# pelinski/TransformerGrooveInfilling

Hardware: AMD Instinct MI355X
Metric: HVO sequences/sec (32-step, d_model=128) per train step (higher is better)
Workload: dtype f32; 1 GPU; BASELINE configs[1]: InfillingClosedHH_training.yaml + overrides d_model=128/4 heads/3 layers, dim_feedforward=512, bs=64 per GPU, dropout=0.24, SGD lr=0.07, hit_loss_penalty=0.38, S=16, encoder-only; global_batch=64, parallelism=dp1, hipgraph=False

## Files before the change

transformergrooveinfilling_amd/csrc/gt_seq.h:

```cpp
#pragma once
#include "gt_seq_api.h"
#include <type_traits>

#ifdef GT_SEQ_STAMPS
#define GT_STAMP(i) do { if (blockIdx.x == 0 && threadIdx.x == 0) reinterpret_cast<long long*>(a.ws + a.stamps)[(i)] = (long long)__builtin_amdgcn_s_memtime(); } while (0)
__shared__ long long* gt_sub_ptr;
#define GT_SUBSTAMP(i) do { if (threadIdx.x == 0 && gt_sub_ptr) gt_sub_ptr[(i)] = (long long)__builtin_amdgcn_s_memtime(); } while (0)
#define GT_SUBWAIT() asm volatile("s_waitcnt vmcnt(0) lgkmcnt(0)" ::: "memory")
#define GT_SUBSET(on) do { if (threadIdx.x == 0) gt_sub_ptr = ((on) && blockIdx.x == 0) ? reinterpret_cast<long long*>(a.ws + a.stamps) + 200 : nullptr; } while (0)
#define GT_WGSTAMP(k) do { if (threadIdx.x == 0 && a.phase == 1 && blockIdx.x < 512) { long long* q_ = reinterpret_cast<long long*>(a.ws + a.stamps) + 1024 + 4 * blockIdx.x + 2 * (k); \
    q_[0] = (long long)__builtin_amdgcn_s_memtime(); q_[1] = (long long)__builtin_amdgcn_s_memrealtime(); } } while (0)
#else
#define GT_WGSTAMP(k) do { } while (0)
#define GT_STAMP(i) do { } while (0)
#define GT_SUBSTAMP(i) do { } while (0)
#define GT_SUBWAIT() do { } while (0)
#define GT_SUBSET(on) do { } while (0)
#endif

#define GT_SEQ_WAVES 8
#define GT_SEQ_NT (GT_SEQ_WAVES * 64)
#define GT_SEQ_NT_WG GT_SEQ_NT
#include "gt_seq_wg.h"

// ... 78 lines not shown
      w[j] = __hip_atomic_load(slot + j * GT_SEQ_NT + tid, __ATOMIC_RELAXED, __HIP_MEMORY_SCOPE_AGENT);
      ok = ok && (uint32_t)(w[j] >> 32) == GT_XTAG;
    }
    if (__all(ok)) break;
    if (spins == 0 && __hip_atomic_load(err, __ATOMIC_RELAXED, __HIP_MEMORY_SCOPE_AGENT) != 0u) spins = spin_max;
    if (++spins > spin_max) { if ((tid & 63) == 0) __hip_atomic_store(err, 1u, __ATOMIC_RELAXED, __HIP_MEMORY_SCOPE_AGENT); break; }
    __builtin_amdgcn_s_sleep(1);
  }
#pragma unroll
  for (int j = 0; j < 4; ++j) __hip_atomic_store(slot + j * GT_SEQ_NT + tid, 0ull, __ATOMIC_RELAXED, __HIP_MEMORY_SCOPE_AGENT);
#endif
  return f32x4{gt_u2f((uint32_t)w[0]), gt_u2f((uint32_t)w[1]), gt_u2f((uint32_t)w[2]), gt_u2f((uint32_t)w[3])};
}


template <bool BKM, bool VEC>
__device__ __forceinline__ void seq_ldb(float (&b)[4], const float* __restrict__ W, const int ldw, const int n, const int N, const int k,
                                        const int K, const float* zp) {
  if (!BKM && VEC) {
    const float4 v = *reinterpret_cast<const float4*>((n < N && k < K) ? W + (size_t)n * ldw + k : zp);
    b[0] = v.x; b[1] = v.y; b[2] = v.z; b[3] = v.w;
  } else if (!BKM) {
#pragma unroll
    for (int j = 0; j < 4; ++j) b[j] = *((n < N && k + j < K) ? W + (size_t)n * ldw + k + j : zp);
  } else {
#pragma unroll
    for (int j = 0; j < 4; ++j) b[j] = *((n < N && k + j < K) ? W + (size_t)(k + j) * ldw + n : zp);
  }
}
template <bool HALF>
__device__ __forceinline__ void seq_mma(f32x4& acc0, f32x4& acc1, const float (&b)[4], const float* sA, const int lda, const int l16, const int k) {
  const float4 a0 = *reinterpret_cast<const float4*>(sA + l16 * lda + k);
  acc0 = GT_MFMA16(b[0], a0.x, acc0); acc0 = GT_MFMA16(b[1], a0.y, acc0); acc0 = GT_MFMA16(b[2], a0.z, acc0); acc0 = GT_MFMA16(b[3], a0.w, acc0);
  if (!HALF) {
    const float4 a1 = *reinterpret_cast<const float4*>(sA + (16 + l16) * lda + k);
    acc1 = GT_MFMA16(b[0], a1.x, acc1); acc1 = GT_MFMA16(b[1], a1.y, acc1); acc1 = GT_MFMA16(b[2], a1.z, acc1); acc1 = GT_MFMA16(b[3], a1.w, acc1);
  }
}
template <bool BKM, bool VEC, int NK, bool HALF, typename Epi>
__device__ __forceinline__ void seq_mm_edge(const float* sA, const int lda, const int K, const float* __restrict__ W, const int ldw, const int N,
                                            const float* __restrict__ bias, const int wave, const int lane, const float* zp, Epi epi) {
  const int l16 = lane & 15, lg = lane >> 4;
  const int n0 = wave * 16;
  if (n0 >= N) return;
  float b[NK][4], bi[4];
#pragma unroll
  for (int u = 0; u < NK; ++u) { if (16 * u < K) seq_ldb<BKM, VEC>(b[u], W, ldw, n0 + l16, N, 16 * u + 4 * lg, K, zp); }
#pragma unroll
  for (int r = 0; r < 4; ++r) bi[r] = *((bias != nullptr && n0 + 4 * lg + r < N) ? bias + n0 + 4 * lg + r : zp);
  f32x4 acc0 = f32x4{0.f, 0.f, 0.f, 0.f}, acc1 = f32x4{0.f, 0.f, 0.f, 0.f};
#pragma unroll
  for (int u = 0; u < NK; ++u) { if (16 * u < K) seq_mma<HALF>(acc0, acc1, b[u], sA, lda, l16, 16 * u + 4 * lg); }
  epi(n0, acc0, acc1, bi);
}

template <int NK> struct SeqB { float4 v[NK]; };
template <int NK, bool FULL = false>
__device__ __forceinline__ void seq_b_load(SeqB<NK>& b, const float* __restrict__ Wp, const int nkt, const int t, const int u0, const int nk,
                                           const int lane) {
  const float* p = Wp + (unsigned)(((t * nkt + u0) * 64 + lane) * 4);
#pragma unroll
  for (int u = 0; u < NK; ++u) { if (FULL || u < nk) b.v[u] = *reinterpret_cast<const float4*>(p + 256 * u); }
}
#ifdef GT_SEQ_TU_FWD
__global__ __launch_bounds__(256) void seq_pack_kernel(SeqArgs a) {
  const int lane = threadIdx.x & 63, l16 = lane & 15, lg = lane >> 4;
  const int d = a.d, F = a.F, d16 = d >> 4, f16 = F >> 4;
  const int nf0 = 3 * d16 * d16, nf1 = d16 * d16, nf2 = f16 * d16, T = nf0 + nf1 + 2 * nf2;
  const int g = blockIdx.x * 4 + (threadIdx.x >> 6);
  if (g >= 2 * a.L * T) return;
  const int pack = g / (a.L * T), r = g % (a.L * T), l = r / T;
  int f = r % T, R, C;
  int64_t src, moff;
  if (f < nf0) { src = a.p0.in_w; R = 3 * d; C = d; moff = 0; }
  else if (f < nf0 + nf1) { f -= nf0; src = a.p0.out_w; R = d; C = d; moff = (int64_t)3 * d * d; }
  else if (f < nf0 + nf1 + nf2) { f -= nf0 + nf1; src = a.p0.w1; R = F; C = d; moff = (int64_t)4 * d * d; }
  else { f -= nf0 + nf1 + nf2; src = a.p0.w2; R = d; C = F; moff = (int64_t)4 * d * d + (int64_t)d * F; }
  const float* W = a.prm + src + (int64_t)l * a.pstride;
  float4 v;
  if (pack == 0) {
    const int nkt = C >> 4, t = f / nkt, u = f % nkt;
    v = *reinterpret_cast<const float4*>(W + (size_t)(16 * t + l16) * C + 16 * u + 4 * lg);
  } else {
    const int nkt = R >> 4, t = f / nkt, u = f % nkt;
    const float* p = W + (size_t)(16 * u + 4 * lg) * C + 16 * t + l16;
    v = make_float4(p[0], p[C], p[2 * (size_t)C], p[3 * (size_t)C]);
  }
  *reinterpret_cast<float4*>(a.ws + (pack ? a.pack_b : a.pack_f) + (int64_t)l * a.kstride + moff + (int64_t)f * 256 + lane * 4) = v;
}

struct SeqUpd { float* prm; float* g; float* m; float* v; int64_t n; const gt_step_state* st; int algo, step_advanced, nblk_a; const unsigned* err; };
__device__ __forceinline__ float seq_upd_elem(const SeqUpd& u, const int64_t i, const float w, const float g, const float k, const float b1,
                                              const float b2, const float step_size, const float inv_sqrt_bc2, const float gs, const float eps,
                                              const bool skip) {
  if (skip) return w;
  if (u.algo == 0) return w - k * g;
  const float gi = g * gs;
  const float mi = b1 * u.m[i] + (1.0f - b1) * gi;
  const float vi = b2 * u.v[i] + (1.0f - b2) * gi * gi;
  u.m[i] = mi; u.v[i] = vi;
  return w - step_size * mi / (sqrtf(vi) * inv_sqrt_bc2 + eps);
}
__global__ __launch_bounds__(256) void seq_update_pack_kernel(SeqArgs a, SeqUpd u) {
  __shared__ float tr[4][16][17];
  const int lane = threadIdx.x & 63, wave = threadIdx.x >> 6, l16 = lane & 15, lg = lane >> 4;
  const float k = u.st->lr * u.st->grad_scale;
// ... 867 lines not shown
  if (tid >= 2 * nkrow * H) return;
  const int pb = tid & 1, jb = krow0 + (tid >> 1) % nkrow, hb = (tid >> 1) / nkrow;
  const float msc = dk.thr ? dk.scale : 1.0f;
  const int i0 = 16 * pb;
  const float* qp = sQ + hb * HD + i0 * ldq;
  const float* dop = sDO + hb * HD + i0 * lddo;
  const float* rdp = srd + hb * 32 + i0;
  const uint32_t* mwp = reinterpret_cast<const uint32_t*>(srd) + H * 32 + hb * 32 + i0;
  const float* pim = sImg + (4 * pb) * 2048 + (4 * hb) * 32 + 4 * ((jb >> 2) ^ (hb & 7)) + (jb & 3);
  const int hx = hb >> 3;
  const SeqHv<HD> v = seq_hv_ld<HD>(sQ + jb * ldq + 2 * d + hb * HD);
  const uint32_t allk = dk.thr ? 0u : 1u;
#pragma unroll
  for (int i = 0; i < 16; ++i) {
    const float pi = pim[(i >> 2) * 2048 + ((i & 3) ^ hx) * 32];
    const float mk = (((mwp[i] >> jb) | allk) & 1u) ? msc : 0.f;
    const SeqHv<HD> dO = seq_hv_ld<HD>(dop + i * lddo), qi = seq_hv_ld<HD>(qp + i * ldq);
    const float pm = pi * mk, g = pi * (seq_hv_dot<HD>(dO, v) * mk - rdp[i]) * scale;
#pragma unroll
    for (int c = 0; c < HD; ++c) { G.dvv.v[c] += pm * dO.v[c]; G.dkk.v[c] += g * qi.v[c]; }
    if ((i & 3) == 3) { GT_SCHED_FENCE() }
  }
#pragma unroll
  for (int c = 0; c < HD; ++c) { G.dvv.v[c] += seq_lane_swap1(G.dvv.v[c]); G.dkk.v[c] += seq_lane_swap1(G.dkk.v[c]); }
}
template <int HD>
__device__ __forceinline__ void seq_attn_bwd_small_store(const SeqAttnSmallG<HD>& G, float* sQ, const int ldq, const int d, const int H,
                                                         const int krow0, const int nkrow, const int tid) {
  if (tid < 32 * H) {
    const int ha = tid % H, ia = tid / H;
#pragma unroll
    for (int c = 0; c < HD; ++c) sQ[ia * ldq + ha * HD + c] = G.dq.v[c];
  }
  if (tid < 2 * nkrow * H) {
    const int pb = tid & 1, jb = krow0 + (tid >> 1) % nkrow, hb = (tid >> 1) / nkrow;
    float* dst = sQ + jb * ldq + (pb ? 2 * d : d) + hb * HD;
#pragma unroll
    for (int c = 0; c < HD; ++c) dst[c] = pb ? G.dvv.v[c] : G.dkk.v[c];
  }
}

__device__ __forceinline__ int seq_vblock(const int bid, const int nper, const int B) {
  if ((B & 7) != 0 || bid >= nper * B) return bid;
  const int xcd = bid & 7, slot = bid >> 3;
  return ((slot / nper) * 8 + xcd) * nper + slot % nper;
}

template <int DP> struct SeqGeo {
  static constexpr int SX = DP + 8, SH = GT_SEQ_FMAX + 8, SQ = 3 * DP + 8, SRS = DP + 8, RP = DP == 32 ? 8 : DP == 64 ? 2 : 1, CW = DP / 16;
  static constexpr int TILE = 32 * SX, QKV = 32 * SQ, FFN = 32 * SH, RES = RP * 32 * SRS, NK = DP / 16;
  static constexpr int UNI = QKV > FFN ? QKV : FFN;
};
template <int DP> struct SeqFwdLds { static constexpr int N = 3 * SeqGeo<DP>::TILE + SeqGeo<DP>::RES + SeqGeo<DP>::UNI; };
template <int DP, int HDC, bool EXACT, bool SPLIT, bool QUAD = false>
__device__ __forceinline__ bool seq_fwd_body(const SeqArgs& a, float* const lds) {
  static_assert(!QUAD || (SPLIT && EXACT && DP == 128), "QUAD: the SPLIT kernels of d_model 128");
  using G = SeqGeo<DP>;
  constexpr int SX = G::SX, SH = G::SH, SQ = G::SQ, SRS = G::SRS, CW = G::CW, NK = G::NK;
  constexpr int HD = SeqHd<HDC>::HD;
  constexpr bool PAD = SeqHd<HDC>::PAD;
  constexpr bool HALF = SPLIT;
  constexpr int NH = HALF ? 1 : 2, NROW = HALF ? 16 : 32;
  float* const sX = lds; float* const sX1 = sX + G::TILE; float* const sC = sX1 + G::TILE; float* const sR = sC + G::TILE; float* const sU = sR + G::RES;
  float* const sQ = sU;
  float* const sH = sU;
  const int tid = threadIdx.x, lane = tid & 63, wave = tid >> 6, l16 = lane & 15, lg = lane >> 4;
  const int vb = (SPLIT && !QUAD) ? seq_vblock((int)blockIdx.x, 2, a.B) : (int)blockIdx.x;
  const int cpart = QUAD ? (vb & 1) : 0;
  const int half_id = QUAD ? (vb >> 1) : vb;
  const int b = SPLIT ? half_id >> 1 : (int)blockIdx.x, rb = SPLIT ? 16 * (half_id & 1) : 0;
  const bool sv0 = !QUAD || cpart == 0, sv1 = !QUAD || cpart == 1;
  const int d = EXACT ? DP : a.d, F = a.F;
  const size_t r0 = (size_t)b * 32;
  const float* const zp = gt_zero_ptr();
  const float* prm = a.prm;
  float* ws = a.ws;
  const SeqDropK dk = seq_dropk(a);
  const uint32_t idxd = (uint32_t)(r0 * d), idxf = (uint32_t)(r0 * F);
  const float ascale = 1.0f / sqrtf((float)a.hd);
  constexpr bool PF32 = SPLIT && !QUAD && EXACT && (DP == 32 || DP == 64);
  constexpr bool PFLN = PF32;
  SeqB<NK> ipre = SeqB<NK>();
  float4 ipre_b = make_float4(0.f, 0.f, 0.f, 0.f);
  bool have_ipre = false;
  auto load_rows = [&](float* dst, const int str, const float* src, const int ncol, const int rb_, const int nrows) {
    const int q4 = ncol >> 2;
    for (int e = tid; e < nrows * q4; e += GT_SEQ_NT) {
      const int r = rb_ + e / q4, c = (e % q4) * 4;
      *reinterpret_cast<float4*>(dst + r * str + c) = *reinterpret_cast<const float4*>(src + (unsigned)(r * ncol + c));
    }
  };

  auto input_layer = [&](auto all_tag) {
    constexpr bool HF = HALF && !decltype(all_tag)::value;
    constexpr int NHX = HF ? 1 : 2, NRX = HF ? 16 : 32;
    const int rbx = HF ? rb : 0;
    for (int e = tid; e < NRX * 32; e += GT_SEQ_NT) {
      const int r = rbx + (e >> 5), c = e & 31;
      sC[r * SX + c] = *(c < a.S ? a.xin + (r0 + r) * a.S + c : zp);
    }
    GT_BARRIER();
    GT_STAMP(1);
    const uint32_t key = seq_key(dk, GT_SITE_PE_ENC);
    float* ga0 = ws + a.a0 + r0 * d;
    float* gx0 = ws + a.x0 + r0 * d;
    seq_mm_edge<false, false, 2, HF>(sC + rbx * SX, SX, a.S, prm + a.in_w, a.S, d, prm + a.in_b, wave, lane, zp,
                                     [&](int n0, const f32x4& c0, const f32x4& c1, const float (&bi)[4]) {
#pragma unroll
      for (int h2 = 0; h2 < NHX; ++h2) {
// ... 163 lines not shown
    GT_BARRIER();
    GT_SUBSET(false);
    GT_STAMP(sb + 5);
    if constexpr (QUAD) {
      seq_tile_out_cols(wl + a.w0.hact + r0 * F, F, sH, SH, fc0, fcn, tid, rb, NROW);
      f32x4 acc0 = f32x4{0.f, 0.f, 0.f, 0.f}, acc1 = acc0;
      seq_mm_krange<true>(acc0, acc1, sH + rb * SH + l16 * SH + 4 * lg, SH, kf_w2, nkf, wave, kq0, kq0 + (nkf >> 1), lane, pre2, b2pre);
      GT_STAMP(300 + 4 * l);
      unsigned long long* const xq = reinterpret_cast<unsigned long long*>(ws + a.xchg) + 8;
      const bool last = l + 1 == a.L;
      const bool fz = a.fuse_b0 != 0;
      if (!last || cpart == 1 || fz) seq_xchg_put(xq + (size_t)vb * GT_XCHG_WG_GRANULES, acc0, tid);
      if (last && cpart == 1 && !fz) return true;
      *reinterpret_cast<float4*>(&sR[(16 * cpart + l16) * SRS + 16 * wave + 4 * lg]) = make_float4(acc0[0], acc0[1], acc0[2], acc0[3]);
      GT_STAMP(301 + 4 * l);
      const f32x4 oth = seq_xchg_get(xq + (size_t)(vb ^ 1) * GT_XCHG_WG_GRANULES, tid, reinterpret_cast<unsigned*>(ws + a.xchg), a.spin_max);
      GT_STAMP(302 + 4 * l);
      *reinterpret_cast<float4*>(&sR[(16 * (1 - cpart) + l16) * SRS + 16 * wave + 4 * lg]) = make_float4(oth[0], oth[1], oth[2], oth[3]);
    } else {
      seq_tile_out(wl + a.w0.hact + r0 * F, sH, SH, F, tid, rb, NROW);
      seq_mm_splitk<HALF>(sH + rb * SH, SH, F, kf_w2, d, sR + rb * SRS, SRS, wave, lane, pre2, b2pre);
    }
    GT_BARRIER();
    GT_STAMP(sb + 6);
    {
      const uint32_t key = seq_key(dk, site0 + GT_SITE_DROPF);
      const float* b2 = pl + a.p0.b2;
      const int parts = seq_splitk_parts(d);
      seq_ln_fwd<DP, HALF>([&](int row, int c0, float (&z)[CW]) {
        float bi[CW], xr[CW];
        if constexpr (QUAD) {
          float u[CW];
          SeqVec<CW>::ld(z, &sR[(row - rb) * SRS + c0]); SeqVec<CW>::ld(u, &sR[(16 + row - rb) * SRS + c0]);
#pragma unroll
          for (int e = 0; e < CW; ++e) z[e] += u[e];
        } else {
          seq_parts_sum<CW>(z, sR, SRS, parts, row, c0);
        }
        SeqVec<CW>::ld(xr, &sX1[row * SX + c0]);
        if constexpr (PFLN) {
#pragma unroll
          for (int e = 0; e < CW; ++e) bi[e] = ln2p.bi[e];
        } else SeqVec<CW>::ld(bi, b2 + c0);
#pragma unroll
        for (int e = 0; e < CW; ++e) z[e] = (z[e] + bi[e]) * seq_dmul(dk, key, idxd + (uint32_t)(row * d + c0 + e)) + xr[e];
      }, sX, SX, d, pl + a.p0.n2w, pl + a.p0.n2b, (sv0 || fzl) ? wl + a.w0.xout + r0 * d : nullptr, wl + a.w0.xhat2 + r0 * d, wl + a.w0.rstd2 + r0, tid, rb,
         PFLN ? &ln2p : nullptr);
    }
    GT_BARRIER();
    GT_STAMP(sb + 7);
    return false;
  };
  auto output_layer = [&]() {
    seq_ln_fwd<DP, HALF>([&](int row, int c0, float (&z)[CW]) { SeqVec<CW>::ld(z, &sX[row * SX + c0]); }, sC, SX, d, prm + a.encn_w, prm + a.encn_b,
                         ws + a.memory + r0 * d, ws + a.enc_xhat + r0 * d, ws + a.enc_rstd + r0, tid, rb);
    GT_BARRIER();
    seq_mm_edge<false, true, NK, HALF>(sC + rb * SX, SX, d, prm + a.out_w, d, GT_TGT, prm + a.out_b, wave, lane, zp,
                                       [&](int n0, const f32x4& c0, const f32x4& c1, const float (&bi)[4]) {
#pragma unroll
      for (int h2 = 0; h2 < NH; ++h2) {
        const f32x4& c = h2 ? c1 : c0;
#pragma unroll
        for (int r = 0; r < 4; ++r) {
          const int col = n0 + 4 * lg + r;
          if (col < GT_TGT) {
            float v = c[r] + bi[r];
            if (col >= 2 * GT_VOICES) v = 0.5f * tanhf(v);
            else if (col >= GT_VOICES) v = gt_sigmoid(v);
            a.hvo[(r0 + rb + 16 * h2 + l16) * GT_TGT + col] = v;
            sR[(rb + 16 * h2 + l16) * 28 + col] = v;
          }
        }
      }
    });
    if (a.loss_y == nullptr) return;
    const unsigned lwg_n = QUAD ? gridDim.x >> 1 : gridDim.x, lwg_id = QUAD ? (unsigned)half_id : blockIdx.x;
    GT_BARRIER();
    float* red = sX1;
    const float invM = 1.0f / (float)(a.B * 32);
    float bce = 0.f, mv = 0.f, mo = 0.f, ok = 0.f;
    if (tid < NROW * GT_VOICES) {
      const int row = rb + tid / GT_VOICES, j = tid % GT_VOICES;
      const size_t base = (r0 + row) * GT_TGT + j;
      float gh, gv, go;
      gt_loss_elem<true>(sR[row * 28 + j], sR[row * 28 + j + GT_VOICES], sR[row * 28 + j + 2 * GT_VOICES], a.loss_y[base],
                         a.loss_y[base + GT_VOICES], a.loss_y[base + 2 * GT_VOICES], a.loss_penalty, invM, bce, mv, mo, ok, gh, gv, go);
      ws[a.dlogits + base] = gh; ws[a.dlogits + base + GT_VOICES] = gv; ws[a.dlogits + base + 2 * GT_VOICES] = go;
    }
    bce = gt_wave_sum(bce); mv = gt_wave_sum(mv); mo = gt_wave_sum(mo); ok = gt_wave_sum(ok);
    if (lane == 0) { red[wave * 4 + 0] = bce; red[wave * 4 + 1] = mv; red[wave * 4 + 2] = mo; red[wave * 4 + 3] = ok; }
    GT_BARRIER();
    if (tid == 0 && cpart != 0) red[32] = 0.0f;
    if (tid == 0 && cpart == 0) {
#pragma unroll
      for (int q = 0; q < 4; ++q) {
        float t = red[q];
        for (int w = 1; w < GT_SEQ_WAVES; ++w) t += red[w * 4 + q];
        gt_pub_store(a.loss_part + lwg_id * 4 + q, t);
      }
      const unsigned t = gt_pub_ticket(a.loss_ticket);
      red[32] = (t == lwg_n - 1) ? 1.0f : 0.0f;
    }
    GT_BARRIER();
    if (red[32] == 0.0f) return;
    if (wave < 4) {
      float acc = 0.f;
      for (unsigned bk = lane; bk < lwg_n; bk += 64) acc += gt_pub_load(a.loss_part + bk * 4 + wave);
      acc = gt_wave_sum(acc);
      if (lane == 0) red[40 + wave] = acc * invM;
    }
    GT_BARRIER();
    if (tid == 0) {
      const float b_ = red[40], v_ = red[41], o_ = red[42];
      a.loss_stats[0] = b_ + v_ + o_;
      a.loss_stats[1] = red[43] * (1.0f / GT_VOICES);
      a.loss_stats[2] = 0.f;
      a.loss_stats[3] = b_; a.loss_stats[4] = v_; a.loss_stats[5] = o_; a.loss_stats[6] = 0.f; a.loss_stats[7] = 0.f;
      *a.loss_ticket = 0u;
    }
  };

#ifdef GT_SEQ_STAMPS
  GT_SUBSET(false);
  GT_BARRIER();
#endif
  typedef std::true_type AllRows;
  typedef std::false_type OwnRows;
  if (!SPLIT) {
    GT_STAMP(0);
    input_layer(OwnRows{});
    for (int l = 0; l < a.L; ++l) { in_proj(l, OwnRows{}); (void)layer_rest(l, true); }
    output_layer();
    GT_STAMP(2 + 10 * a.L);
  } else {
    const int l = a.phase;
    if constexpr (QUAD) {
      if (l < 0) {
        input_layer(OwnRows{});
        in_proj(0, OwnRows{});
        seq_tile_out_cols(ws + a.w0.qkv + r0 * 3 * d, 3 * d, sQ, SQ, cpart * (3 * d / 2), 3 * d / 2, tid, rb, NROW);
        return false;
      }
    }
    const bool pro = QUAD && a.quad_pro != 0;
    GT_STAMP(60 + 2 * (l + 1));
    GT_WGSTAMP(0);
    if (l == 0 && !pro) {
      input_layer(AllRows{});
      in_proj(0, AllRows{});
    } else {
      load_rows(sX, SX, ws + (l == 0 ? a.x0 : (int64_t)(l - 1) * a.wstride + a.w0.xout) + r0 * d, d, rb, NROW);
      {
        const float* gq = ws + (int64_t)l * a.wstride + a.w0.qkv + r0 * 3 * d;
        const int q4k = (2 * d) >> 2, q4q = d >> 2;
        for (int e = tid; e < 32 * q4k; e += GT_SEQ_NT) {
          const int r = e / q4k, c = d + (e % q4k) * 4;
          *reinterpret_cast<float4*>(sQ + r * SQ + c) = *reinterpret_cast<const float4*>(gq + (unsigned)(r * 3 * d + c));
        }
        for (int e = tid; e < NROW * q4q; e += GT_SEQ_NT) {
          const int r = rb + e / q4q, c = (e % q4q) * 4;
          *reinterpret_cast<float4*>(sQ + r * SQ + c) = *reinterpret_cast<const float4*>(gq + (unsigned)(r * 3 * d + c));
        }
      }
      GT_BARRIER();
    }
    GT_STAMP(2 + 10 * l + 1);
    if (layer_rest(l, l == 0 && !pro)) return false;
    if (l + 1 < a.L) {
      in_proj(l + 1, OwnRows{});
      float* const gq = ws + (int64_t)(l + 1) * a.wstride + a.w0.qkv + r0 * 3 * d;
      if (QUAD) seq_tile_out_cols(gq, 3 * d, sQ, SQ, cpart * (3 * d / 2), 3 * d / 2, tid, rb, NROW);
      else seq_tile_out(gq, sQ, SQ, 3 * d, tid, rb, NROW);
    } else {
      output_layer();
    }
    GT_WGSTAMP(1);
    GT_STAMP(61 + 2 * (l + 1));
  }
  return true;
}
template <int DP, int HDC, bool EXACT, bool SPLIT, bool QUAD = false>
__global__ __launch_bounds__(GT_SEQ_NT) void seq_fwd_kernel(SeqArgs a) {
  __shared__ __attribute__((aligned(16))) float lds[SeqFwdLds<DP>::N];
  (void)seq_fwd_body<DP, HDC, EXACT, SPLIT, QUAD>(a, lds);
}

struct SeqRdPre { float4 a0, c0, a1, c1; };
template <int DP> struct SeqBwdLds {
  using G = SeqGeo<DP>;
  static constexpr int U = DP > 64 ? G::UNI : G::QKV + G::FFN, P = 2 * GT_SEQ_WAVES * DP;
  static constexpr int N = 3 * G::TILE + G::RES + U + P + 32 * GT_SEQ_WAVES / 2;
};
template <int DP, int HDC, bool EXACT, bool SPLIT, bool QUAD = false>
__device__ __forceinline__ void seq_bwd_body(const SeqArgs& a, float* const lds) {
  static_assert(!QUAD || (SPLIT && EXACT && DP == 128), "QUAD: the SPLIT kernels of d_model 128");
  using G = SeqGeo<DP>;
  constexpr int SX = G::SX, SH = G::SH, SQ = G::SQ, SRS = G::SRS, CW = G::CW, NK = G::NK;
  constexpr int HD = SeqHd<HDC>::HD;
  constexpr bool PAD = SeqHd<HDC>::PAD;
  constexpr bool HALF = SPLIT;
  constexpr int NROW = HALF ? 16 : 32;
  constexpr bool ALIAS = DP > 64;
  float* const sZ = lds; float* const sDZ = sZ + G::TILE; float* const sC = sDZ + G::TILE; float* const sR = sC + G::TILE;
  float* const sU = sR + G::RES; float* const sP = sU + SeqBwdLds<DP>::U; float* const srd = sP + SeqBwdLds<DP>::P;
  float* const sQ = sU;
  float* const sH = ALIAS ? sU : sU + G::QKV;
  const int tid = threadIdx.x, lane = tid & 63, wave = tid >> 6, l16 = lane & 15, lg = lane >> 4;
  const int vb = (SPLIT && !QUAD) ? seq_vblock((int)blockIdx.x, 2, a.B) : (int)blockIdx.x;
  const int cpart = QUAD ? (vb & 1) : 0, half_id = QUAD ? (vb >> 1) : vb;
  const int b = SPLIT ? half_id >> 1 : (int)blockIdx.x, rb = SPLIT ? 16 * (half_id & 1) : 0;
  const bool sv0 = !QUAD || cpart == 0;
  const int d = EXACT ? DP : a.d, F = a.F;
  const size_t r0 = (size_t)b * 32;
  if constexpr (SPLIT && DP == 128 && !QUAD) {
    if (a.grd != nullptr && (int)blockIdx.x >= a.nseq) {
      static_assert(SeqBwdLds<DP>::U >= GT_WG_LDS && SeqBwdLds<DP>::P >= 8 * 64, "rider LDS");
      seq_wg_riders(a, a.phase, (int)blockIdx.x - a.nseq, (int)gridDim.x - a.nseq, sU, sP, tid);
      return;
    }
  }
  const float* const zp = gt_zero_ptr();
  const float* prm = a.prm;
  float* ws = a.ws;
  const SeqDropK dk = seq_dropk(a);
  const uint32_t idxd = (uint32_t)(r0 * d);
  const float mscale = dk.thr ? dk.scale : 1.0f;
  const float ascale = 1.0f / sqrtf((float)a.hd);
  auto part_at = [&](int job) { return ws + a.ln_part + (int64_t)job * a.ln_part_stride + (size_t)(QUAD ? half_id : (int)blockIdx.x) * 2 * d; };
  auto load_rows = [&](float* dst, const int str, const float* src, const int ncol, const int rb_, const int nrows) {
    const int q4 = ncol >> 2;
    for (int e = tid; e < nrows * q4; e += GT_SEQ_NT) {
      const int r = rb_ + e / q4, c = (e % q4) * 4;
      *reinterpret_cast<float4*>(dst + r * str + c) = *reinterpret_cast<const float4*>(src + (unsigned)(r * ncol + c));
    }
  };

  auto prologue = [&]() {
    for (int e = tid; e < NROW * 32; e += GT_SEQ_NT) {
      const int r = rb + (e >> 5), c = e & 31;
      sC[r * SX + c] = *(c < GT_TGT ? ws + a.dlogits + (r0 + r) * GT_TGT + c : zp);
    }
    if (!SPLIT) load_rows(sH, SH, ws + a.w0.hact + (int64_t)(a.L - 1) * a.wstride + r0 * F, F, 0, 32);
    GT_BARRIER();
    seq_mm_edge<true, true, 2, HALF>(sC + rb * SX, SX, GT_TGT, prm + a.out_w, d, d, nullptr, wave, lane, zp,
                                     [&](int n0, const f32x4& c0, const f32x4& c1, const float (&)[4]) {
      const int col = n0 + 4 * lg;
      *reinterpret_cast<float4*>(&sZ[(rb + l16) * SX + col]) = make_float4(c0[0], c0[1], c0[2], c0[3]);
      if (!HALF) *reinterpret_cast<float4*>(&sZ[(16 + l16) * SX + col]) = make_float4(c1[0], c1[1], c1[2], c1[3]);
    });
    GT_BARRIER();
    {
      SeqDropK nd = dk; nd.thr = 0u;
      seq_ln_bwd<DP, HALF>([&](int row, int c0, float (&g)[CW]) { SeqVec<CW>::ld(g, &sZ[row * SX + c0]); }, sZ, sC, SX, d, ws + a.enc_xhat + r0 * d,
                           ws + a.enc_rstd + r0, prm + a.encn_w, nd, 0u, 0u, nullptr, nullptr, sP, tid, rb);
    }
    GT_BARRIER();
    if (sv0) seq_ln_part<DP, HALF>(sP, part_at(0), d, tid);
    GT_BARRIER();
    GT_STAMP(101);
  };
  constexpr bool PFB = SPLIT && !QUAD && EXACT && (DP == 32 || DP == 64);
  constexpr bool PFBLN = PFB;
  SeqLnBwdPre<CW> lb2p, lb1p;
  bool have_lbp = false;
  constexpr int F2T = GT_SEQ_FMAX / (QUAD ? 256 : 128);
  SeqTilesAll<NK, F2T> f2p;
  auto chain = [&](const int l, const bool fromg) {
    const float* pl = prm + (int64_t)l * a.pstride;
    const float* kb = ws + a.pack_b + (int64_t)l * a.kstride;
    const float* kb_out = kb + 3 * d * d, *kb_w1 = kb + 4 * d * d, *kb_w2 = kb_w1 + d * F;
    float* wl = ws + (int64_t)l * a.wstride;
    float* tl = ws + (int64_t)l * a.tstride;
    const int site0 = GT_SITE_LAYER0 + 8 * l, jb = 1 + 2 * (a.L - 1 - l);
    const int sb = 102 + 10 * (a.L - 1 - l);
    static_assert(16 * GT_SEQ_FMAX / 4 <= 4 * GT_SEQ_NT, "four 16-byte loads per thread cover the 16 x F tile");
    if constexpr (PFB) seq_tiles_all_load<NK, F2T, false>(f2p, kb_w2, d, F, nullptr, wave, lane);
    float4 hp0 = make_float4(0.f, 0.f, 0.f, 0.f), hp1 = hp0, hp2 = hp0, hp3 = hp0;
    const int fc0 = QUAD ? cpart * (F >> 1) : 0, fcn = QUAD ? F >> 1 : F;
    const int hq4 = fcn >> 2, hn = 16 * hq4;
    auto hoff = [&](const int u) { const int e = tid + u * GT_SEQ_NT, ec = e < hn ? e : hn - 1; return (unsigned)((rb + ec / hq4) * F + fc0 + (ec % hq4) * 4); };
    if (SPLIT) {
      const float* src = wl + a.w0.hact + r0 * F;
      hp0 = *reinterpret_cast<const float4*>(src + hoff(0)); hp1 = *reinterpret_cast<const float4*>(src + hoff(1));
      hp2 = *reinterpret_cast<const float4*>(src + hoff(2)); hp3 = *reinterpret_cast<const float4*>(src + hoff(3));
    } else if (ALIAS && !fromg) {
      load_rows(sH, SH, wl + a.w0.hact + r0 * F, F, rb, NROW);
    }
    {
      const uint32_t key = seq_key(dk, site0 + GT_SITE_DROPF);
      const int parts = seq_splitk_parts(d);
      seq_ln_bwd<DP, HALF>([&](int row, int c0, float (&g)[CW]) {
        if (fromg) SeqVec<CW>::ld(g, &sZ[row * SX + c0]);
        else {
          float r[CW];
          seq_parts_sum<CW>(g, sR, SRS, parts, row, c0); SeqVec<CW>::ld(r, &sDZ[row * SX + c0]);
#pragma unroll
          for (int e = 0; e < CW; ++e) g[e] += r[e];
        }
      }, sDZ, sC, SX, d, wl + a.w0.xhat2 + r0 * d, wl + a.w0.rstd2 + r0, pl + a.p0.n2w, dk, key, idxd, sv0 ? tl + a.t0.dzA + r0 * d : nullptr,
                           (dk.thr && sv0) ? tl + a.t0.dzAm + r0 * d : nullptr, sP, tid, rb, (PFBLN && have_lbp) ? &lb2p : nullptr);
    }
    if (SPLIT) {
      auto hst = [&](const int u, const float4& v) { const int e = tid + u * GT_SEQ_NT; if (e < hn) *reinterpret_cast<float4*>(sH + (rb + e / hq4) * SH + fc0 + (e % hq4) * 4) = v; };
      hst(0, hp0); hst(1, hp1); hst(2, hp2); hst(3, hp3);
    }
    GT_BARRIER();
    GT_STAMP(sb);
    if (sv0) seq_ln_part<DP, HALF>(sP, part_at(jb), d, tid);
    auto ffn2d_epi = [&](int n0, const f32x4& c0, const f32x4& c1, const float4&) {
      const int col = fc0 + n0 + 4 * lg;
#pragma unroll
      for (int h2 = 0; h2 < (HALF ? 1 : 2); ++h2) {
        float* hp = &sH[(rb + 16 * h2 + l16) * SH + col];
        const f32x4& c = h2 ? c1 : c0;
        const float4 ha = *reinterpret_cast<const float4*>(hp);
        *reinterpret_cast<float4*>(hp) = make_float4(ha.x != 0.f ? c[0] * mscale : 0.f, ha.y != 0.f ? c[1] * mscale : 0.f,
                                                     ha.z != 0.f ? c[2] * mscale : 0.f, ha.w != 0.f ? c[3] * mscale : 0.f);
      }
    };
    if constexpr (PFB) seq_mm_tiles_all<NK, F2T, HALF>(sC + rb * SX, SX, d, fcn, wave, lane, f2p, ffn2d_epi);
    else seq_mm_tiles<NK, F2T, EXACT, HALF>(sC + rb * SX, SX, d, kb_w2 + (size_t)(fc0 >> 4) * (d >> 4) * 256, fcn, nullptr, wave, lane, ffn2d_epi);
    const int nkf = F >> 4, kq0 = QUAD ? cpart * (nkf >> 1) : 0;
    const bool pre1 = QUAD ? ((nkf >> 1) & 7) == 0 : (SPLIT && seq_splitk_pre_ok(F, d));
    SeqB<8> b1pre = SeqB<8>();
    if (pre1) {
      if (QUAD) seq_b_load<8, true>(b1pre, kb_w1, nkf, wave, kq0, 8, lane);
      else b1pre = seq_splitk_first(kb_w1, F, d, wave, lane);
    }
    GT_BARRIER();
    GT_STAMP(sb + 1);
    SeqB<NK> bodpre = SeqB<NK>();
    if constexpr (PFB) bodpre = seq_tiles_first<NK>(kb_out, d, d, wave, lane);
    if constexpr (QUAD) {
      seq_tile_out_cols(tl + a.t0.dhid + r0 * F, F, sH, SH, fc0, fcn, tid, rb, NROW);
      f32x4 acc0 = f32x4{0.f, 0.f, 0.f, 0.f}, acc1 = acc0;
      seq_mm_krange<true>(acc0, acc1, sH + rb * SH + l16 * SH + 4 * lg, SH, kb_w1, nkf, wave, kq0, kq0 + (nkf >> 1), lane, pre1, b1pre);
      const int64_t xoff = a.fuse_b0 ? a.xchg_b : a.xchg;
      unsigned long long* const xq = reinterpret_cast<unsigned long long*>(ws + xoff) + 8;
      seq_xchg_put(xq + (size_t)vb * GT_XCHG_WG_GRANULES, acc0, tid);
      *reinterpret_cast<float4*>(&sR[(16 * cpart + l16) * SRS + 16 * wave + 4 * lg]) = make_float4(acc0[0], acc0[1], acc0[2], acc0[3]);
      const f32x4 oth = seq_xchg_get(xq + (size_t)(vb ^ 1) * GT_XCHG_WG_GRANULES, tid, reinterpret_cast<unsigned*>(ws + a.xchg), a.spin_max);
      *reinterpret_cast<float4*>(&sR[(16 * (1 - cpart) + l16) * SRS + 16 * wave + 4 * lg]) = make_float4(oth[0], oth[1], oth[2], oth[3]);
    } else {
      seq_tile_out(tl + a.t0.dhid + r0 * F, sH, SH, F, tid, rb, NROW);
      seq_mm_splitk<HALF>(sH + rb * SH, SH, F, kb_w1, d, sR + rb * SRS, SRS, wave, lane, pre1, b1pre);
    }
    GT_BARRIER();
    GT_STAMP(sb + 2);
    if (!SPLIT) load_rows(sQ, SQ, wl + a.w0.qkv + r0 * 3 * d, 3 * d, 0, 32);
    {
      const uint32_t key = seq_key(dk, site0 + GT_SITE_DROP1);
      const int parts = seq_splitk_parts(d);
      seq_ln_bwd<DP, HALF>([&](int row, int c0, float (&g)[CW]) {
        float r[CW];
        if constexpr (QUAD) {
          float u[CW];
          SeqVec<CW>::ld(g, &sR[(row - rb) * SRS + c0]); SeqVec<CW>::ld(u, &sR[(16 + row - rb) * SRS + c0]);
#pragma unroll
          for (int e = 0; e < CW; ++e) g[e] += u[e];
        } else {
          seq_parts_sum<CW>(g, sR, SRS, parts, row, c0);
        }
        SeqVec<CW>::ld(r, &sDZ[row * SX + c0]);
#pragma unroll
        for (int e = 0; e < CW; ++e) g[e] += r[e];
      }, sDZ, sC, SX, d, wl + a.w0.xhat1 + r0 * d, wl + a.w0.rstd1 + r0, pl + a.p0.n1w, dk, key, idxd, sv0 ? tl + a.t0.dzB + r0 * d : nullptr,
                           (dk.thr && sv0) ? tl + a.t0.dzBm + r0 * d : nullptr, sP, tid, rb, (PFBLN && have_lbp) ? &lb1p : nullptr);
    }
    GT_BARRIER();
    GT_STAMP(sb + 3);
    if (sv0) seq_ln_part<DP, HALF>(sP, part_at(jb + 1), d, tid);
    if (DP <= 64 && !SPLIT) seq_mm_square(sC, SX, d, kb_out, sZ, SX, wave, lane);
    else if constexpr (QUAD)
      seq_mm_tiles<NK, 1, EXACT, true>(sC + rb * SX, SX, d, kb_out + (size_t)cpart * (d >> 5) * NK * 256, d >> 1, nullptr, wave, lane,
                                       [&](int n0, const f32x4& c0, const f32x4&, const float4&) {
        *reinterpret_cast<float4*>(&sZ[(rb + l16) * SX + cpart * (d >> 1) + n0 + 4 * lg]) = make_float4(c0[0], c0[1], c0[2], c0[3]);
      });
    else
      seq_mm_tiles<NK, 1, EXACT, HALF>(sC + rb * SX, SX, d, kb_out, d, nullptr, wave, lane, [&](int n0, const f32x4& c0, const f32x4& c1, const float4&) {
        *reinterpret_cast<float4*>(&sZ[(rb + l16) * SX + n0 + 4 * lg]) = make_float4(c0[0], c0[1], c0[2], c0[3]);
        if (!HALF) *reinterpret_cast<float4*>(&sZ[(16 + l16) * SX + n0 + 4 * lg]) = make_float4(c1[0], c1[1], c1[2], c1[3]);
      }, PFB, bodpre);
    GT_BARRIER();
    GT_STAMP(sb + 4);
  };
  auto chain_prefetch = [&](const int l) {
    if constexpr (PFBLN) {
      if (l > 0) {
        const float* wp = ws + (int64_t)(l - 1) * a.wstride;
        const float* pp = prm + (int64_t)(l - 1) * a.pstride;
        seq_ln_bwd_pre<CW>(lb2p, d, wp + a.w0.xhat2 + r0 * d, wp + a.w0.rstd2 + r0, pp + a.p0.n2w, tid, rb);
        seq_ln_bwd_pre<CW>(lb1p, d, wp + a.w0.xhat1 + r0 * d, wp + a.w0.rstd1 + r0, pp + a.p0.n1w, tid, rb);
        have_lbp = true;
      }
    }
  };
  SeqPRow prow = SeqPRow();
  constexpr bool RD2 = 32 * (DP / 4) > GT_SEQ_NT;
  auto rd_tile_request = [&](const float* gd, const float* gc) {
    static_assert(G::RES >= 32 * DP && 32 * (DP / 4) <= 2 * GT_SEQ_NT, "row sums of every head in sR; two 16-byte pieces per thread cover a tile");
    SeqRdPre p = SeqRdPre();
    const int q4 = d >> 2, n = 32 * q4;
// ... 139 lines not shown
    prologue();
    chain(a.L - 1, true);
    seq_tile_out(ws + a.dctx + r0 * d, sZ, SX, d, tid, rb, NROW);
    GT_STAMP(161);
  } else {
    const int l = a.L - a.phase;
    GT_STAMP(160 + 2 * a.phase);
    const int64_t hand = (int64_t)a.B * 32 * d;
    const float* const gdctx = ws + a.dctx + ((a.phase - 1) & 1) * hand + r0 * d;
    const float* const gctx = ws + (int64_t)l * a.wstride + a.w0.ctx + r0 * d;
    bool va = false;
    if constexpr (VATTN) {
      va = a.hd == DP / 16 && a.H == 16;
      if (va)
        prow = seq_attn_bwd_small_load(ws + (int64_t)l * a.wstride + a.w0.P + (size_t)(b * a.H) * 1024,
                                       reinterpret_cast<const uint32_t*>(ws + a.amask + (int64_t)l * a.amask_stride) + b * a.H * 32, tid);
    }
    SeqRdPre rdp = SeqRdPre();
    if constexpr (OWN && !PAD) rdp = rd_tile_request(gdctx, gctx);
    else if constexpr (OWN) rd_small_stage(gdctx, gctx);
    else load_rows(sZ, SX, gdctx, d, 0, 32);
    load_rows(sQ, SQ, ws + (int64_t)l * a.wstride + a.w0.qkv + r0 * 3 * d, 3 * d, 0, 32);
    load_rows(sDZ, SX, ws + (int64_t)l * a.tstride + a.t0.dzB + r0 * d, d, rb, NROW);
    chain_prefetch(l);
    if constexpr (OWN && !PAD) rd_tile_finish(rdp);
    GT_BARRIER();
    GT_STAMP(400 + 4 * a.phase);
    SeqB<8> bqpre;
    if constexpr (VATTN) {
      if (va) bqpre = attn_bwd(l, std::true_type{});
      else bqpre = attn_bwd(l, std::false_type{});
    } else {
      bqpre = attn_bwd(l, std::false_type{});
    }
    inproj_dgrad(l, bqpre);
    if (l > 0) {
      chain(l - 1, false);
      seq_tile_out(ws + a.dctx + (a.phase & 1) * hand + r0 * d, sZ, SX, d, tid, rb, NROW);
    } else {
      input_bwd();
    }
    GT_STAMP(161 + 2 * a.phase);
  }
}
template <int DP, int HDC, bool EXACT, bool SPLIT, bool QUAD = false>
__global__ __launch_bounds__(GT_SEQ_NT) void seq_bwd_kernel(SeqArgs a) {
  __shared__ __attribute__((aligned(16))) float lds[SeqBwdLds<DP>::N];
  seq_bwd_body<DP, HDC, EXACT, SPLIT, QUAD>(a, lds);
}
template <int HDC>
__global__ __launch_bounds__(GT_SEQ_NT) void seq_fb_kernel(SeqArgs a) {
  constexpr int N = SeqBwdLds<128>::N > SeqFwdLds<128>::N ? SeqBwdLds<128>::N : SeqFwdLds<128>::N;
  __shared__ __attribute__((aligned(16))) float lds[N];
  if (!seq_fwd_body<128, HDC, true, true, true>(a, lds)) return;
  __syncthreads();
  SeqArgs b = a;
  b.phase = 0;
  seq_bwd_body<128, 32, true, true, true>(b, lds);
}
```

transformergrooveinfilling_amd/csrc/gt_seq_api.h:

```cpp
#pragma once
#include "gt_common.h"

#define GT_SEQ_FMAX 512
#ifndef GT_XCHG_SPIN_MAX
#define GT_XCHG_SPIN_MAX (1 << 22)
#endif
struct SeqLayerP { int64_t in_w, in_b, out_w, out_b, w1, b1, w2, b2, n1w, n1b, n2w, n2b; };
struct SeqLayerW { int64_t qkv, P, ctx, xhat1, rstd1, x1, hact, xhat2, rstd2, xout; };
struct SeqTmp { int64_t dzA, dzAm, dzB, dzBm, dhid, dqkv; };
struct SeqArgs {
  const float* prm; float* ws; const float* pe; const float* xin; float* hvo;
  int B, S, d, F, H, L, hd;
  const gt_step_state* st; uint32_t thr; float dscale;
  SeqLayerP p0; int64_t pstride;
  SeqLayerW w0; int64_t wstride;
  SeqTmp t0; int64_t tstride;
  int64_t in_w, in_b, encn_w, encn_b, out_w, out_b;
  int64_t x0, a0, memory, enc_xhat, enc_rstd, dlogits, da0;
  int64_t ln_part, ln_part_stride;
  int64_t stamps;
  int64_t pack_f, pack_b, kstride;
  int64_t dctx;
  int64_t amask, amask_stride;
  int64_t xchg;
  int64_t xchg_b; int fuse_b0;
  int spin_max;
  int quad_pro;
  int phase;
  const float* loss_y; float loss_penalty; float* loss_stats; float* loss_part; unsigned* loss_ticket;
  float* grd;
  int nseq;
  int wg_accumulate;
  int ride_last_k;
  int out_early;
  int tail_phase;
  int tail_ksplit;
  int ln_nwg;
  gt_step_state* bump;
};
static inline int gt_seq_wg_tiles(int rows, int cols) { return ((rows + 31) / 32) * ((cols + 63) / 64); }
void gt_seq_launch_pack(const SeqArgs& a, unsigned nblocks, hipStream_t s);
void gt_seq_launch_update_pack(const SeqArgs& a, int algo, float* params, float* grads, float* m, float* v, int64_t n, const gt_step_state* st,
                               int step_advanced, hipStream_t s);
void gt_seq_launch_fwd(const SeqArgs& a, int d_model, int hc, bool split, unsigned nblocks, hipStream_t s, bool quad = false);
static inline int64_t gt_seq_xchg_floats(int batch) { return 16 + (int64_t)4 * batch * 4 * 512 * 2; }
void gt_seq_launch_fb(const SeqArgs& a, unsigned nblocks, hipStream_t s);
void gt_seq_launch_bwd(const SeqArgs& a, int d_model, int hc, bool split, unsigned nblocks, hipStream_t s, bool quad = false);
void gt_seq_launch_tail(const SeqArgs& a, unsigned nblocks, hipStream_t s);
void gt_seq_launch_fwd64(const SeqArgs& a, int hc, unsigned nblocks, hipStream_t s);
void gt_seq_launch_bwd64(const SeqArgs& a, int hc, unsigned nblocks, hipStream_t s);
```

Baseline: 327,000 sequences/s.

## Hand off forward outputs to backward in LDS within fused fwd-bwd kernel

In the fused forward+backward launch, the output-layer weights and loss targets are prefetched before the final layernorm. Loss gradients are written straight into shared memory so the backward prologue can skip reloading dlogits and the last layer's activations from global memory. The cross-workgroup loss reduction moves into the backward pass, finished by the last ticket holder, instead of blocking at the end of forward. LN-backward prefetches are also issued early. The cost is more register pressure and a more intricate handover protocol between the two phases.

```diff
diff --git a/transformergrooveinfilling_amd/csrc/gt_seq.h b/transformergrooveinfilling_amd/csrc/gt_seq.h
--- a/transformergrooveinfilling_amd/csrc/gt_seq.h
+++ b/transformergrooveinfilling_amd/csrc/gt_seq.h
@@ -154,6 +154,29 @@
 #pragma unroll
   for (int u = 0; u < NK; ++u) { if (16 * u < K) seq_mma<HALF>(acc0, acc1, b[u], sA, lda, l16, 16 * u + 4 * lg); }
   epi(n0, acc0, acc1, bi);
+}
+template <int NK> struct SeqEdgeB { float b[NK][4], bi[4]; };
+template <bool BKM, bool VEC, int NK>
+__device__ __forceinline__ void seq_mm_edge_load(SeqEdgeB<NK>& e, const int K, const float* __restrict__ W, const int ldw, const int N,
+                                                 const float* __restrict__ bias, const int wave, const int lane, const float* zp) {
+  const int l16 = lane & 15, lg = lane >> 4;
+  const int n0 = wave * 16;
+  if (n0 >= N) return;
+#pragma unroll
+  for (int u = 0; u < NK; ++u) { if (16 * u < K) seq_ldb<BKM, VEC>(e.b[u], W, ldw, n0 + l16, N, 16 * u + 4 * lg, K, zp); }
+#pragma unroll
+  for (int r = 0; r < 4; ++r) e.bi[r] = *((bias != nullptr && n0 + 4 * lg + r < N) ? bias + n0 + 4 * lg + r : zp);
+}
+template <int NK, bool HALF, typename Epi>
+__device__ __forceinline__ void seq_mm_edge_run(const SeqEdgeB<NK>& e, const float* sA, const int lda, const int K, const int N, const int wave,
+                                                const int lane, Epi epi) {
+  const int l16 = lane & 15, lg = lane >> 4;
+  const int n0 = wave * 16;
+  if (n0 >= N) return;
+  f32x4 acc0 = f32x4{0.f, 0.f, 0.f, 0.f}, acc1 = f32x4{0.f, 0.f, 0.f, 0.f};
+#pragma unroll
+  for (int u = 0; u < NK; ++u) { if (16 * u < K) seq_mma<HALF>(acc0, acc1, e.b[u], sA, lda, l16, 16 * u + 4 * lg); }
+  epi(n0, acc0, acc1, e.bi);
 }
 
 template <int NK> struct SeqB { float4 v[NK]; };
@@ -1127,9 +1150,10 @@
   static constexpr int UNI = QKV > FFN ? QKV : FFN;
 };
 template <int DP> struct SeqFwdLds { static constexpr int N = 3 * SeqGeo<DP>::TILE + SeqGeo<DP>::RES + SeqGeo<DP>::UNI; };
-template <int DP, int HDC, bool EXACT, bool SPLIT, bool QUAD = false>
+template <int DP, int HDC, bool EXACT, bool SPLIT, bool QUAD = false, bool FB = false>
 __device__ __forceinline__ bool seq_fwd_body(const SeqArgs& a, float* const lds) {
   static_assert(!QUAD || (SPLIT && EXACT && DP == 128), "QUAD: the SPLIT kernels of d_model 128");
+  static_assert(!FB || QUAD, "FB: the fused launch of the QUAD schedule");
   using G = SeqGeo<DP>;
   constexpr int SX = G::SX, SH = G::SH, SQ = G::SQ, SRS = G::SRS, CW = G::CW, NK = G::NK;
   constexpr int HD = SeqHd<HDC>::HD;
@@ -1399,11 +1423,19 @@
     return false;
   };
   auto output_layer = [&]() {
+    SeqEdgeB<NK> ob;
+    float ly0 = 0.f, ly1 = 0.f, ly2 = 0.f;
+    if constexpr (FB) {
+      seq_mm_edge_load<false, true, NK>(ob, d, prm + a.out_w, d, GT_TGT, prm + a.out_b, wave, lane, zp);
+      if (tid < NROW * GT_VOICES) {
+        const float* yp = a.loss_y + (r0 + rb + tid / GT_VOICES) * GT_TGT + tid % GT_VOICES;
+        ly0 = yp[0]; ly1 = yp[GT_VOICES]; ly2 = yp[2 * GT_VOICES];
+      }
+    }
     seq_ln_fwd<DP, HALF>([&](int row, int c0, float (&z)[CW]) { SeqVec<CW>::ld(z, &sX[row * SX + c0]); }, sC, SX, d, prm + a.encn_w, prm + a.encn_b,
                          ws + a.memory + r0 * d, ws + a.enc_xhat + r0 * d, ws + a.enc_rstd + r0, tid, rb);
     GT_BARRIER();
-    seq_mm_edge<false, true, NK, HALF>(sC + rb * SX, SX, d, prm + a.out_w, d, GT_TGT, prm + a.out_b, wave, lane, zp,
-                                       [&](int n0, const f32x4& c0, const f32x4& c1, const float (&bi)[4]) {
+    auto out_epi = [&](int n0, const f32x4& c0, const f32x4& c1, const float (&bi)[4]) {
 #pragma unroll
       for (int h2 = 0; h2 < NH; ++h2) {
         const f32x4& c = h2 ? c1 : c0;
@@ -1419,7 +1451,9 @@
           }
         }
       }
-    });
+    };
+    if constexpr (FB) seq_mm_edge_run<NK, HALF>(ob, sC + rb * SX, SX, d, GT_TGT, wave, lane, out_epi);
+    else seq_mm_edge<false, true, NK, HALF>(sC + rb * SX, SX, d, prm + a.out_w, d, GT_TGT, prm + a.out_b, wave, lane, zp, out_epi);
     if (a.loss_y == nullptr) return;
     const unsigned lwg_n = QUAD ? gridDim.x >> 1 : gridDim.x, lwg_id = QUAD ? (unsigned)half_id : blockIdx.x;
     GT_BARRIER();
@@ -1430,13 +1464,21 @@
       const int row = rb + tid / GT_VOICES, j = tid % GT_VOICES;
       const size_t base = (r0 + row) * GT_TGT + j;
       float gh, gv, go;
-      gt_loss_elem<true>(sR[row * 28 + j], sR[row * 28 + j + GT_VOICES], sR[row * 28 + j + 2 * GT_VOICES], a.loss_y[base],
-                         a.loss_y[base + GT_VOICES], a.loss_y[base + 2 * GT_VOICES], a.loss_penalty, invM, bce, mv, mo, ok, gh, gv, go);
+      if constexpr (!FB) { ly0 = a.loss_y[base]; ly1 = a.loss_y[base + GT_VOICES]; ly2 = a.loss_y[base + 2 * GT_VOICES]; }
+      gt_loss_elem<true>(sR[row * 28 + j], sR[row * 28 + j + GT_VOICES], sR[row * 28 + j + 2 * GT_VOICES], ly0, ly1, ly2, a.loss_penalty, invM,
+                         bce, mv, mo, ok, gh, gv, go);
       ws[a.dlogits + base] = gh; ws[a.dlogits + base + GT_VOICES] = gv; ws[a.dlogits + base + 2 * GT_VOICES] = go;
+      if constexpr (FB) { sC[row * SX + j] = gh; sC[row * SX + j + GT_VOICES] = gv; sC[row * SX + j + 2 * GT_VOICES] = go; }
+    }
+    if constexpr (FB) {
+      constexpr int ZC = 32 - GT_TGT;
+      const int t = tid - NROW * GT_VOICES;
+      if (t >= 0 && t < NROW * ZC) sC[(rb + t / ZC) * SX + GT_TGT + t % ZC] = 0.f;
     }
     bce = gt_wave_sum(bce); mv = gt_wave_sum(mv); mo = gt_wave_sum(mo); ok = gt_wave_sum(ok);
     if (lane == 0) { red[wave * 4 + 0] = bce; red[wave * 4 + 1] = mv; red[wave * 4 + 2] = mo; red[wave * 4 + 3] = ok; }
     GT_BARRIER();
+    if constexpr (FB) return;
     if (tid == 0 && cpart != 0) red[32] = 0.0f;
     if (tid == 0 && cpart == 0) {
 #pragma unroll
@@ -1525,6 +1567,27 @@
     GT_STAMP(61 + 2 * (l + 1));
   }
   return true;
+}
+__device__ __forceinline__ void seq_loss_finish(const SeqArgs& a, const unsigned tick, const unsigned lwg_n, const int lane) {
+  if (__shfl((lane == 0 && tick == lwg_n - 1) ? 1.0f : 0.0f, 0) == 0.0f) return;
+  const float invM = 1.0f / (float)(a.B * 32);
+  float s[4] = {0.f, 0.f, 0.f, 0.f};
+  for (unsigned bk = lane; bk < lwg_n; bk += 64) {
+    float v[4];
+#pragma unroll
+    for (int q = 0; q < 4; ++q) v[q] = gt_pub_load(a.loss_part + bk * 4 + q);
+#pragma unroll
+    for (int q = 0; q < 4; ++q) s[q] += v[q];
+  }
+#pragma unroll
+  for (int q = 0; q < 4; ++q) s[q] = gt_wave_sum(s[q]) * invM;
+  if (lane == 0) {
+    a.loss_stats[0] = s[0] + s[1] + s[2];
+    a.loss_stats[1] = s[3] * (1.0f / GT_VOICES);
+    a.loss_stats[2] = 0.f;
+    a.loss_stats[3] = s[0]; a.loss_stats[4] = s[1]; a.loss_stats[5] = s[2]; a.loss_stats[6] = 0.f; a.loss_stats[7] = 0.f;
+    *a.loss_ticket = 0u;
+  }
 }
 template <int DP, int HDC, bool EXACT, bool SPLIT, bool QUAD = false>
 __global__ __launch_bounds__(GT_SEQ_NT) void seq_fwd_kernel(SeqArgs a) {
@@ -1582,13 +1645,25 @@
     }
   };
 
+  unsigned tick = ~0u;
+  constexpr bool PFQ = QUAD;
+  SeqLnBwdPre<CW> lbep, lbqp;
   auto prologue = [&]() {
-    for (int e = tid; e < NROW * 32; e += GT_SEQ_NT) {
-      const int r = rb + (e >> 5), c = e & 31;
-      sC[r * SX + c] = *(c < GT_TGT ? ws + a.dlogits + (r0 + r) * GT_TGT + c : zp);
-    }
-    if (!SPLIT) load_rows(sH, SH, ws + a.w0.hact + (int64_t)(a.L - 1) * a.wstride + r0 * F, F, 0, 32);
-    GT_BARRIER();
+    if constexpr (PFQ) {
+      const float* wq = ws + (int64_t)(a.L - 1) * a.wstride;
+      seq_ln_bwd_pre<CW>(lbep, d, ws + a.enc_xhat + r0 * d, ws + a.enc_rstd + r0, prm + a.encn_w, tid, rb);
+      seq_ln_bwd_pre<CW>(lbqp, d, wq + a.w0.xhat2 + r0 * d, wq + a.w0.rstd2 + r0, prm + (int64_t)(a.L - 1) * a.pstride + a.p0.n2w, tid, rb);
+    }
+    bool din = false;
+    if constexpr (QUAD) din = a.fb_handover != 0;
+    if (!din) {
+      for (int e = tid; e < NROW * 32; e += GT_SEQ_NT) {
+        const int r = rb + (e >> 5), c = e & 31;
+        sC[r * SX + c] = *(c < GT_TGT ? ws + a.dlogits + (r0 + r) * GT_TGT + c : zp);
+      }
+      if (!SPLIT) load_rows(sH, SH, ws + a.w0.hact + (int64_t)(a.L - 1) * a.wstride + r0 * F, F, 0, 32);
+      GT_BARRIER();
+    }
     seq_mm_edge<true, true, 2, HALF>(sC + rb * SX, SX, GT_TGT, prm + a.out_w, d, d, nullptr, wave, lane, zp,
                                      [&](int n0, const f32x4& c0, const f32x4& c1, const float (&)[4]) {
       const int col = n0 + 4 * lg;
@@ -1596,10 +1671,20 @@
       if (!HALF) *reinterpret_cast<float4*>(&sZ[(16 + l16) * SX + col]) = make_float4(c1[0], c1[1], c1[2], c1[3]);
     });
     GT_BARRIER();
+    if constexpr (QUAD) {
+      if (a.fb_handover != 0 && cpart == 0 && wave == GT_SEQ_WAVES - 1) {
+        if (lane < 4) {
+          float t = sDZ[lane];
+          for (int w = 1; w < GT_SEQ_WAVES; ++w) t += sDZ[w * 4 + lane];
+          gt_pub_store(a.loss_part + half_id * 4 + lane, t);
+        }
+        if (lane == 0) tick = gt_pub_ticket(a.loss_ticket);
+      }
+    }
     {
       SeqDropK nd = dk; nd.thr = 0u;
       seq_ln_bwd<DP, HALF>([&](int row, int c0, float (&g)[CW]) { SeqVec<CW>::ld(g, &sZ[row * SX + c0]); }, sZ, sC, SX, d, ws + a.enc_xhat + r0 * d,
-                           ws + a.enc_rstd + r0, prm + a.encn_w, nd, 0u, 0u, nullptr, nullptr, sP, tid, rb);
+                           ws + a.enc_rstd + r0, prm + a.encn_w, nd, 0u, 0u, nullptr, nullptr, sP, tid, rb, PFQ ? &lbep : nullptr);
     }
     GT_BARRIER();
     if (sv0) seq_ln_part<DP, HALF>(sP, part_at(0), d, tid);
@@ -1626,7 +1711,9 @@
     const int fc0 = QUAD ? cpart * (F >> 1) : 0, fcn = QUAD ? F >> 1 : F;
     const int hq4 = fcn >> 2, hn = 16 * hq4;
     auto hoff = [&](const int u) { const int e = tid + u * GT_SEQ_NT, ec = e < hn ? e : hn - 1; return (unsigned)((rb + ec / hq4) * F + fc0 + (ec % hq4) * 4); };
-    if (SPLIT) {
+    bool hin = false;
+    if constexpr (QUAD) hin = a.fb_handover != 0 && fromg;
+    if (SPLIT && !hin) {
       const float* src = wl + a.w0.hact + r0 * F;
       hp0 = *reinterpret_cast<const float4*>(src + hoff(0)); hp1 = *reinterpret_cast<const float4*>(src + hoff(1));
       hp2 = *reinterpret_cast<const float4*>(src + hoff(2)); hp3 = *reinterpret_cast<const float4*>(src + hoff(3));
@@ -1645,9 +1732,9 @@
           for (int e = 0; e < CW; ++e) g[e] += r[e];
         }
       }, sDZ, sC, SX, d, wl + a.w0.xhat2 + r0 * d, wl + a.w0.rstd2 + r0, pl + a.p0.n2w, dk, key, idxd, sv0 ? tl + a.t0.dzA + r0 * d : nullptr,
-                           (dk.thr && sv0) ? tl + a.t0.dzAm + r0 * d : nullptr, sP, tid, rb, (PFBLN && have_lbp) ? &lb2p : nullptr);
-    }
-    if (SPLIT) {
+                           (dk.thr && sv0) ? tl + a.t0.dzAm + r0 * d : nullptr, sP, tid, rb, PFQ ? &lbqp : (PFBLN && have_lbp) ? &lb2p : nullptr);
+    }
+    if (SPLIT && !hin) {
       auto hst = [&](const int u, const float4& v) { const int e = tid + u * GT_SEQ_NT; if (e < hn) *reinterpret_cast<float4*>(sH + (rb + e / hq4) * SH + fc0 + (e % hq4) * 4) = v; };
       hst(0, hp0); hst(1, hp1); hst(2, hp2); hst(3, hp3);
     }
@@ -1695,6 +1782,9 @@
     GT_BARRIER();
     GT_STAMP(sb + 2);
     if (!SPLIT) load_rows(sQ, SQ, wl + a.w0.qkv + r0 * 3 * d, 3 * d, 0, 32);
+    if constexpr (QUAD) {
+      if (a.fb_handover != 0 && cpart == 0 && wave == GT_SEQ_WAVES - 1) seq_loss_finish(a, tick, gridDim.x >> 1, lane);
+    }
     {
       const uint32_t key = seq_key(dk, site0 + GT_SITE_DROP1);
       const int parts = seq_splitk_parts(d);
@@ -1940,9 +2030,10 @@
 __global__ __launch_bounds__(GT_SEQ_NT) void seq_fb_kernel(SeqArgs a) {
   constexpr int N = SeqBwdLds<128>::N > SeqFwdLds<128>::N ? SeqBwdLds<128>::N : SeqFwdLds<128>::N;
   __shared__ __attribute__((aligned(16))) float lds[N];
-  if (!seq_fwd_body<128, HDC, true, true, true>(a, lds)) return;
+  if (!seq_fwd_body<128, HDC, true, true, true, true>(a, lds)) return;
   __syncthreads();
   SeqArgs b = a;
   b.phase = 0;
+  b.fb_handover = 1;
   seq_bwd_body<128, 32, true, true, true>(b, lds);
 }
diff --git a/transformergrooveinfilling_amd/csrc/gt_seq_api.h b/transformergrooveinfilling_amd/csrc/gt_seq_api.h
--- a/transformergrooveinfilling_amd/csrc/gt_seq_api.h
+++ b/transformergrooveinfilling_amd/csrc/gt_seq_api.h
@@ -24,6 +24,7 @@
   int64_t amask, amask_stride;
   int64_t xchg;
   int64_t xchg_b; int fuse_b0;
+  int fb_handover;
   int spin_max;
   int quad_pro;
   int phase;
```

After: 334,300 sequences/s (median of 6 runs). +2.2%, better.
